# cc-ai/MUNIT

Measured on AMD Instinct MI355X. Metric: images/sec (gen_update+dis_update) @256x256 bs=8, higher is better.
Workload: dtype f32; 1 GPU; config_256.yaml AdaINGen_double+MsImageDis dis_update+gen_update, 256x256, per-GPU batch 8, fp32; global_batch=8, parallelism=dp1, gen_state=1

## Files before the change

munit_amd/csrc/conv_wgrad.hip:

```cpp
#include "common.h"
#include "wino.h"
#include <cstdlib>
#include <type_traits>

namespace {

struct WgradParams {
  const void* x;
  const void* dy;
  float* slab;
  float* bias_slab;
  int B, H, W, Cin, Hu, Wu, ups;
  int Ho, Wo, Cout;
  int KH, KW, stride, pad, reflect;
  int Ktot, M;
  int pix_per_split;
  long long dy_sb, dy_sh;
  int dy_sw;
  long long dy_off;
  int frame;
  unsigned x_bytes, dy_bytes;
  int ct;
  int x_bf16, dy_bf16;
};
// ... 868 lines not shown
  pl->bias_bytes = align_up((size_t)ns * Cout * sizeof(float), 256);
}

enum WgradForm {
  WG_REFUSED_BF16,
  WG_REFUSED_BF16_X,
  WG_BF16S_128,
  WG_BF16S_256,
  WG_REG_BF16,
  WG_REG_BF16_DY,
  WG_DMA,
  WG_CT1, WG_CT2,
  WG_FAST, WG_ALIGNED, WG_GENERIC
};
struct WgradChoice {
  WgradForm form;
  bool fast;
  long long x_bytes, dy_bytes;
};
WgradChoice wgrad_form(const WgradParams& p, const WgradPlan& pl, bool aligned) {
  WgradChoice c{};
  c.x_bytes = (long long)p.B * p.H * p.W * p.Cin * (p.x_bf16 ? 2 : 4);
  c.dy_bytes = (long long)p.B * p.dy_sb * (p.dy_bf16 ? 2 : 4);
  const bool any_bf16 = p.x_bf16 || p.dy_bf16;
  const bool fast_any = aligned && (p.Cout % 4 == 0) && c.x_bytes < (1ll << 31) && c.dy_bytes < (1ll << 31) &&
                        (long long)p.B * p.H * p.W < (1ll << 23) && (any_bf16 || !MUNIT_ENV_FLAG("MUNIT_DEBUG_NO_FAST_WGRAD"));
  const bool fast = c.fast = fast_any && !p.frame;
  if (any_bf16) {
    const bool dma_ok = p.x_bf16 && p.dy_bf16 && p.Cin % 128 == 0 && p.Cout % 8 == 0 && p.Ho + p.Wo <= DMA_MAX_HW;
    if (!fast && !(fast_any && dma_ok)) c.form = WG_REFUSED_BF16;
    else if (dma_ok && !MUNIT_ENV_FLAG("MUNIT_DEBUG_NO_WGRAD_DMA")) c.form = pl.bc == 256 ? WG_BF16S_256 : WG_BF16S_128;
    else if (p.x_bf16 && p.dy_bf16) c.form = WG_REG_BF16;
    else if (p.dy_bf16) c.form = WG_REG_BF16_DY;
    else c.form = WG_REFUSED_BF16_X;
  } else if (fast && p.ct == 0 && pl.bc == 128 && p.Cin % 128 == 0 && p.Ho + p.Wo <= DMA_MAX_HW &&
             !MUNIT_ENV_FLAG("MUNIT_DEBUG_NO_WGRAD_DMA")) {
    c.form = WG_DMA;
  } else if (fast && p.ct == 1) {
    c.form = WG_CT1;
  } else if (fast && p.ct == 2) {
    c.form = WG_CT2;
  } else {
    c.form = fast ? WG_FAST : aligned ? WG_ALIGNED : WG_GENERIC;
  }
  return c;
}

#define WGRAD_LAUNCH(...)                                                                                         \
  do {                                                                                                            \
    if (pl.bc == 64) hipLaunchKernelGGL((conv_wgrad_kernel<64, __VA_ARGS__>), grid, dim3(WTHR), 0, st, p);        \
    else hipLaunchKernelGGL((conv_wgrad_kernel<128, __VA_ARGS__>), grid, dim3(WTHR), 0, st, p);                   \
  } while (0)

int run_wgrad(WgradParams p, const WgradPlan& pl, bool aligned, float* dw, float* db, float beta, float beta_b,
              void* ws, hipStream_t st) {
  p.slab = reinterpret_cast<float*>(ws);
  p.bias_slab = db ? reinterpret_cast<float*>(reinterpret_cast<char*>(ws) + pl.slab_bytes) : nullptr;
  p.pix_per_split = pl.pix_per_split;
  dim3 grid((unsigned)pl.k_tiles, (unsigned)pl.c_tiles, (unsigned)pl.nsplit);
  const WgradChoice ch = wgrad_form(p, pl, aligned);
  p.x_bytes = ch.fast ? (unsigned)ch.x_bytes : 0u;
  p.dy_bytes = ch.fast ? (unsigned)ch.dy_bytes : 0u;
  switch (ch.form) {
    case WG_REFUSED_BF16:
      munit_set_error("conv2d_wgrad: bf16 tensors need Cin %% 4 == 0, Cout %% 4 == 0, tensors below 2 GiB and B*H*W < 2^23");
      return MUNIT_ERR_ARG;
    case WG_REFUSED_BF16_X:
      munit_set_error("conv2d_wgrad: bf16 x with fp32 dy exists for the 3-channel image head only");
      return MUNIT_ERR_ARG;
    case WG_BF16S_128:
    case WG_BF16S_256: {
      int pps = (cdiv(p.M, pl.nsplit) + BS_WP - 1) / BS_WP * BS_WP;
      p.pix_per_split = pps;
      const int ns = cdiv(p.M, pps);
      if (ch.form == WG_BF16S_256) {
        dim3 g2((unsigned)(p.Ktot / 256), (unsigned)(p.Cout / 256), (unsigned)ns);
        hipLaunchKernelGGL(conv_wgrad_bf16s_kernel<2>, g2, dim3(WTHR), 0, st, p);
      } else {
        dim3 g2((unsigned)cdiv(p.Ktot, 128), (unsigned)cdiv(p.Cout, 128), (unsigned)ns);
        hipLaunchKernelGGL(conv_wgrad_bf16s_kernel<1>, g2, dim3(WTHR), 0, st, p);
      }
      MUNIT_CHECK_LAUNCH("conv_wgrad_bf16s");
      const long long n = (long long)p.Cout * p.Ktot;
      const int blocks = (int)std::min<long long>((n + p.Cout + 255) / 256, 4096);
      hipLaunchKernelGGL(slab_reduce_kernel, dim3(blocks), dim3(256), 0, st, p.slab, dw, n, p.bias_slab, db, p.Cout,
                         ns, beta, beta_b);
      MUNIT_CHECK_LAUNCH("slab_reduce");
      return MUNIT_OK;
    }
    case WG_REG_BF16: WGRAD_LAUNCH(true, true, 1, true, true); break;
    case WG_REG_BF16_DY: WGRAD_LAUNCH(true, true, 0, false, true); break;
    case WG_DMA: hipLaunchKernelGGL((conv_wgrad_kernel<128, true, true, 3>), grid, dim3(WTHR), 0, st, p); break;
    case WG_CT1: WGRAD_LAUNCH(true, true, 1); break;
    case WG_CT2: WGRAD_LAUNCH(true, true, 2); break;
    case WG_FAST: WGRAD_LAUNCH(true, true); break;
    case WG_ALIGNED: WGRAD_LAUNCH(true, false); break;
    case WG_GENERIC: WGRAD_LAUNCH(false, false); break;
  }
  MUNIT_CHECK_LAUNCH("conv_wgrad");
  const long long n = (long long)p.Cout * p.Ktot;
  if (pl.nsplit >= 32 && n + p.Cout <= 64 * 2048) {
    hipLaunchKernelGGL(slab_reduce_wide_kernel, dim3(cdiv(n + p.Cout, 64)), dim3(1024), 0, st, p.slab, dw, n,
                       p.bias_slab, db, p.Cout, pl.nsplit, beta, beta_b);
    MUNIT_CHECK_LAUNCH("slab_reduce_wide");
    return MUNIT_OK;
  }
  const int blocks = (int)std::min<long long>((n + p.Cout + 255) / 256, 4096);
  hipLaunchKernelGGL(slab_reduce_kernel, dim3(blocks), dim3(256), 0, st, p.slab, dw, n, p.bias_slab, db, p.Cout,
                     pl.nsplit, beta, beta_b);
  MUNIT_CHECK_LAUNCH("slab_reduce");
  return MUNIT_OK;
}

bool cin3_padded_ok(const munit_conv_desc* d) {
  return d->Cin == 3 && d->Cout % 4 == 0 && d->upsample == 0 && !MUNIT_ENV_FLAG("MUNIT_DEBUG_NO_CIN3_PAD");
}

bool bf16s_big_tile(const munit_conv_desc* d, int Ho, int Wo) {
  if (MUNIT_ENV_FLAG("MUNIT_DEBUG_NO_WGRAD_BIG_TILE") || MUNIT_ENV_FLAG("MUNIT_DEBUG_NO_WGRAD_DMA")) return false;
  if (d->in_dtype != MUNIT_DTYPE_BF16 || d->out_dtype != MUNIT_DTYPE_BF16) return false;
  if (d->Cin % 256 != 0 || d->Cout % 256 != 0 || Ho + Wo > DMA_MAX_HW) return false;
  const long long tiles = (long long)(d->KH * d->KW * d->Cin / 256) * (d->Cout / 256);
  const long long M = (long long)d->B * Ho * Wo;
  return tiles <= 256 && M * tiles >= 256ll * 1024;
}

bool subpixel_wgrad_ok(const munit_conv_desc* d) {
  const bool f32 = d->in_dtype == MUNIT_DTYPE_F32 && d->out_dtype == MUNIT_DTYPE_F32;
  const bool b16 = d->in_dtype == MUNIT_DTYPE_BF16 && d->out_dtype == MUNIT_DTYPE_BF16 && d->Cin % 128 == 0 &&
                   d->Cout % 8 == 0 && 2 * (d->H + d->W) <= DMA_MAX_HW && !MUNIT_ENV_FLAG("MUNIT_DEBUG_NO_WGRAD_DMA");
  return (f32 || b16) && d->upsample == 1 && d->KH == 5 && d->KW == 5 && d->pad == 2 && d->stride == 1 &&
         d->pad_mode == MUNIT_PAD_REFLECT && d->Cin % 4 == 0 && d->H >= 3 && d->W >= 3 &&
         !MUNIT_ENV_FLAG("MUNIT_DEBUG_NO_SUBPIXEL");
}

struct SubpixelPlan {
  WgradPlan phase, frame;
  size_t dwc_bytes, slab_bytes;
  bool wino;
  int ring;
};
void plan_subpixel(const munit_conv_desc* d, SubpixelPlan* sp) {
  const bool aligned = d->Cin % 4 == 0;
  plan_launch(d->B * (d->H - 2) * (d->W - 2), 9 * d->Cin, d->Cout, aligned, &sp->phase);
  const int Ho = 2 * d->H, Wo = 2 * d->W;
  sp->wino = d->compute == MUNIT_COMPUTE_F32 && d->in_dtype == MUNIT_DTYPE_F32 && d->out_dtype == MUNIT_DTYPE_F32 && d->H >= 4 &&
             d->W >= 4 && munit_wino_wgrad_ok(d->B, d->H, d->W, d->Cin, d->Cout) &&
             (long long)d->B * 4 * d->H * d->W * d->Cout < (1ll << 29);
  sp->ring = sp->wino ? 1 : 2;
  plan_launch(d->B * (2 * sp->ring * Wo + 2 * sp->ring * (Ho - 2 * sp->ring)), 25 * d->Cin, d->Cout, aligned, &sp->frame);
  sp->dwc_bytes = align_up((size_t)4 * d->Cout * 9 * d->Cin * sizeof(float), 256);
  sp->slab_bytes = std::max(sp->phase.slab_bytes + sp->phase.bias_bytes, sp->frame.slab_bytes + sp->frame.bias_bytes);
  if (sp->wino)
    sp->slab_bytes = std::max(sp->slab_bytes, munit_wino_wgrad_workspace((long long)d->B * (d->H / 2) * (d->W / 2), d->Cin, d->Cout, 4));
}

bool wino_wgrad_layer(const munit_conv_desc* d) {
  return d->compute == MUNIT_COMPUTE_F32 && d->in_dtype == MUNIT_DTYPE_F32 && d->out_dtype == MUNIT_DTYPE_F32 && d->KH == 3 &&
         d->KW == 3 && d->stride == 1 && d->pad == 1 && d->upsample == 0 && munit_wino_wgrad_ok(d->B, d->H, d->W, d->Cin, d->Cout);
}
long long s2_tiles(const munit_conv_desc* d) { return (long long)d->B * cdiv(d->H / 2, 3) * cdiv(d->W / 2, 3); }
bool wino_s2_wgrad_layer(const munit_conv_desc* d) {
  return d->compute == MUNIT_COMPUTE_F32 && d->in_dtype == MUNIT_DTYPE_F32 && d->out_dtype == MUNIT_DTYPE_F32 && d->KH == 4 &&
         d->KW == 4 && d->stride == 2 && d->pad == 1 && d->upsample == 0 && d->H >= 4 && d->W >= 4 &&
         munit_wino_wgrad_ok(d->B, d->H, d->W, d->Cin, d->Cout) && !MUNIT_ENV_FLAG("MUNIT_DEBUG_NO_WINOGRAD_S2") &&
         s2_tiles(d) >= (getenv("MUNIT_WINO_S2_MIN_BLOCKS") ? 1 : 512);
}

enum WgradRoute { WGR_WINO_S2, WGR_WINO, WGR_SMALL, WGR_SUBPIXEL, WGR_CIN3, WGR_GENERIC };
struct WgradRoutePlan {
  int rc;
  WgradRoute route;
  int Ho, Wo;
  bool aligned;
  SubpixelPlan sp;
  WgradPlan gen;
  size_t x4_bytes, dw4_bytes;
  size_t ws_bytes;
};
WgradRoutePlan plan_wgrad(const munit_conv_desc* d) {
  WgradRoutePlan pl{};
  pl.rc = munit_conv2d_out_hw(d, &pl.Ho, &pl.Wo);
  if (pl.rc) return pl;
  pl.route = wino_s2_wgrad_layer(d) ? WGR_WINO_S2 : wino_wgrad_layer(d) ? WGR_WINO : munit_small_wgrad_ok(d) ? WGR_SMALL
             : subpixel_wgrad_ok(d) ? WGR_SUBPIXEL : cin3_padded_ok(d) ? WGR_CIN3 : WGR_GENERIC;
  pl.aligned = pl.route == WGR_CIN3 || d->Cin % 4 == 0;
  switch (pl.route) {
    case WGR_WINO_S2: pl.ws_bytes = munit_wino_wgrad_workspace(s2_tiles(d), d->Cin, d->Cout, 4); break;
    case WGR_WINO: pl.ws_bytes = munit_wino_wgrad_workspace((long long)d->B * (d->H / 2) * (d->W / 2), d->Cin, d->Cout, 1); break;
    case WGR_SMALL: pl.ws_bytes = munit_small_wgrad_workspace(d, pl.Ho); break;
    case WGR_SUBPIXEL:
      plan_subpixel(d, &pl.sp);
      pl.ws_bytes = pl.sp.dwc_bytes + pl.sp.slab_bytes;
      break;
    case WGR_CIN3:
      plan_launch(d->B * pl.Ho * pl.Wo, d->KH * d->KW * 4, d->Cout, true, &pl.gen);
      pl.x4_bytes = align_up((size_t)d->B * d->H * d->W * 4 * sizeof(float), 256);
      pl.dw4_bytes = align_up((size_t)d->Cout * d->KH * d->KW * 4 * sizeof(float), 256);
      pl.ws_bytes = pl.x4_bytes + pl.dw4_bytes + pl.gen.slab_bytes + pl.gen.bias_bytes;
      break;
    case WGR_GENERIC:
      plan_launch(d->B * pl.Ho * pl.Wo, d->KH * d->KW * d->Cin, d->Cout, pl.aligned, &pl.gen, bf16s_big_tile(d, pl.Ho, pl.Wo));
      pl.ws_bytes = pl.gen.slab_bytes + pl.gen.bias_bytes;
      break;
  }
  return pl;
}

WgradParams wgrad_params(const munit_conv_desc* d, int Ho, int Wo) {
  WgradParams p{};
  p.x_bf16 = d->in_dtype == MUNIT_DTYPE_BF16; p.dy_bf16 = d->out_dtype == MUNIT_DTYPE_BF16;
  p.B = d->B; p.H = d->H; p.W = d->W; p.Cin = d->Cin;
  p.ups = d->upsample; p.Hu = d->H << p.ups; p.Wu = d->W << p.ups;
  p.Ho = Ho; p.Wo = Wo; p.Cout = d->Cout;
  p.KH = d->KH; p.KW = d->KW; p.stride = d->stride; p.pad = d->pad;
  p.reflect = d->pad_mode == MUNIT_PAD_REFLECT;
  p.ct = d->compute;
  p.Ktot = d->KH * d->KW * d->Cin; p.M = d->B * Ho * Wo;
  p.dy_sw = d->Cout; p.dy_sh = (long long)Wo * d->Cout; p.dy_sb = (long long)Ho * Wo * d->Cout; p.dy_off = 0;
  return p;
}
WinoWgradParams wino_wgrad_params(const munit_conv_desc* d, int Ho, int Wo, WgradRoute route, const void* x, const void* dy) {
  WinoWgradParams q{};
  q.x = reinterpret_cast<const float*>(x); q.dy = reinterpret_cast<const float*>(dy);
  q.x_bytes = (unsigned)((size_t)d->B * d->H * d->W * d->Cin * 4); q.dy_bytes = (unsigned)((size_t)d->B * Ho * Wo * d->Cout * 4);
  q.dy_sw = d->Cout; q.dy_sh = (long long)Wo * d->Cout; q.dy_sb = (long long)Ho * Wo * d->Cout;
  q.B = d->B; q.H = d->H; q.W = d->W; q.Cin = d->Cin; q.Cout = d->Cout;
  q.reflect = d->pad_mode == MUNIT_PAD_REFLECT;
  q.th = d->H / 2; q.tw = d->W / 2; q.phases = 4;
  if (route == WGR_WINO_S2) {
    q.th = cdiv(Ho, 3); q.tw = cdiv(Wo, 3);
    q.s2 = 1; q.Ho = Ho; q.Wo = Wo;
  } else if (route == WGR_WINO) {
    q.xo = -1; q.phases = 1;
  } else {
    q.dy_sw *= 2; q.dy_sh *= 2; q.dy_prow = (long long)Wo * d->Cout; q.dy_pcol = d->Cout;
    q.reflect = 2; q.xo = -1; q.ring_mask = 1;
  }
  return q;
}
WgradParams subpixel_frame_params(const WgradParams& p, const munit_conv_desc* d, const SubpixelPlan& sp, int Ho, int Wo) {
  WgradParams f = p;
  f.frame = sp.ring;
  f.M = d->B * (2 * sp.ring * Wo + 2 * sp.ring * (Ho - 2 * sp.ring));
  return f;
}
WgradParams subpixel_phase_params(const WgradParams& p, const munit_conv_desc* d, int Wo, int ph) {
  const int a = ph >> 1, b = ph & 1;
  WgradParams q = p;
  q.ups = 0; q.Hu = d->H; q.Wu = d->W;
  q.Ho = d->H - 2; q.Wo = d->W - 2;
  q.KH = 3; q.KW = 3; q.pad = 0; q.reflect = 0;
  q.Ktot = 9 * d->Cin; q.M = d->B * q.Ho * q.Wo;
  q.dy_sw = 2 * d->Cout; q.dy_sh = (long long)2 * Wo * d->Cout;
  q.dy_off = ((long long)(2 + a) * Wo + 2 + b) * d->Cout;
  return q;
}
WgradParams cin3_params(const WgradParams& p, const munit_conv_desc* d) {
  WgradParams q = p;
  q.Cin = 4; q.Ktot = d->KH * d->KW * 4; q.x_bf16 = 0;
  q.ct = 0;
  return q;
}
const char* wgrad_refusal(WgradForm f) {
  if (f == WG_REFUSED_BF16) return "refused: bf16 tensors need Cin % 4 == 0, Cout % 4 == 0, tensors below 2 GiB and B*H*W < 2^23";
  if (f == WG_REFUSED_BF16_X) return "refused: bf16 x with fp32 dy exists for the 3-channel image head only";
  return nullptr;
}
}

extern "C" size_t munit_conv2d_wgrad_workspace_bytes(const munit_conv_desc* d) {
  const WgradRoutePlan pl = plan_wgrad(d);
  return pl.rc ? 0 : pl.ws_bytes;
}

extern "C" double munit_conv2d_executed_flops(const munit_conv_desc* d, int pass) {
  if (pass == MUNIT_PASS_FWD || pass == MUNIT_PASS_DGRAD) return munit_igemm_executed_flops(d, pass);
  if (pass != MUNIT_PASS_WGRAD) return 0.0;
  const WgradRoutePlan pl = plan_wgrad(d);
  if (pl.rc) return 0.0;
  const int Ho = pl.Ho, Wo = pl.Wo;
  const double cc = 2.0 * d->Cin * d->Cout;
  switch (pl.route) {
    case WGR_WINO: return cc * d->B * (d->H / 2) * (d->W / 2) * 16;
    case WGR_WINO_S2: return 4 * cc * (double)s2_tiles(d) * 16;
    case WGR_SUBPIXEL:
      if (pl.sp.wino) return cc * d->B * ((double)d->H * d->W * 4 * 4 + (2.0 * Wo + 2.0 * (Ho - 2)) * 25);
      return cc * d->B * ((double)(d->H - 2) * (d->W - 2) * 4 * 9 + (4.0 * Wo + 4.0 * (Ho - 4)) * 25);
    case WGR_CIN3: return 2.0 * 4 * d->Cout * d->B * Ho * Wo * d->KH * d->KW;
    default: return cc * d->B * Ho * Wo * d->KH * d->KW;
  }
}

extern "C" const char* munit_conv2d_kernel_name(const munit_conv_desc* d, int pass) {
  if (pass == MUNIT_PASS_FWD || pass == MUNIT_PASS_DGRAD) return munit_igemm_kernel_name(d, pass);
  if (pass != MUNIT_PASS_WGRAD) return "invalid";
  const WgradRoutePlan pl = plan_wgrad(d);
  if (pl.rc) return "invalid";
  const int Ho = pl.Ho, Wo = pl.Wo;
  const bool x_bf16 = d->in_dtype == MUNIT_DTYPE_BF16, dy_bf16 = d->out_dtype == MUNIT_DTYPE_BF16;
  const WgradParams p = wgrad_params(d, Ho, Wo);
  switch (pl.route) {
    case WGR_WINO_S2:
    case WGR_WINO: {
      const WinoWgradVariant v = munit_wino_wgrad_variant(wino_wgrad_params(d, Ho, Wo, pl.route, nullptr, nullptr));
      if (!v.s2) return v.fast ? "conv_wino_wgrad_kernel<false, true, false> + wino_wgrad_reduce_kernel"
                               : "conv_wino_wgrad_kernel<false, false, false> + wino_wgrad_reduce_kernel";
      return v.fast ? "conv_wino_wgrad_kernel<true, true, false> + wino_wgrad_reduce_kernel"
                    : v.ring ? "conv_wino_wgrad_kernel<true, false, true> + wino_wgrad_reduce_kernel"
                             : "conv_wino_wgrad_kernel<true, false, false> + wino_wgrad_reduce_kernel";
    }
    case WGR_SMALL:
      if (dy_bf16) return "refused: the 3-channel image head has an fp32 dy";
      if (!munit_small_wgrad_pk()) return x_bf16 ? "conv_lanes_wgrad_kernel<bf16_t>" : "conv_lanes_wgrad_kernel";
      return x_bf16 ? "conv_lanes_wgrad_pk_kernel<bf16_t>" : "conv_lanes_wgrad_pk_kernel";
    case WGR_SUBPIXEL: {
      if (pl.sp.wino) return "conv_wino_wgrad_kernel<false, ., true> x4 sub-pixel phases + frame + reduce";
      const WgradForm fr = wgrad_form(subpixel_frame_params(p, d, pl.sp, Ho, Wo), pl.sp.frame, pl.aligned).form;
      const WgradForm ph = wgrad_form(subpixel_phase_params(p, d, Wo, 0), pl.sp.phase, pl.aligned).form;
      if (wgrad_refusal(fr)) return wgrad_refusal(fr);
      if (wgrad_refusal(ph)) return wgrad_refusal(ph);
      if (ph == WG_BF16S_128 && fr == WG_BF16S_128) return "conv_wgrad_bf16s_kernel<1> x4 sub-pixel phases + frame";
      if (x_bf16 || dy_bf16) return "invalid";
      if (ph == WG_CT1) return "conv_wgrad_kernel<.., 1> x4 sub-pixel phases + fp32 frame";
      if (ph == WG_CT2) return "conv_wgrad_kernel<.., 2> x4 sub-pixel phases + fp32 frame";
      return "conv_wgrad_kernel x4 sub-pixel phases + frame";
    }
    case WGR_CIN3:
      if (x_bf16) return "refused: 3-channel inputs are fp32";
      break;
    case WGR_GENERIC: break;
  }
  const WgradForm f = wgrad_form(pl.route == WGR_CIN3 ? cin3_params(p, d) : p, pl.gen, pl.aligned).form;
  if (wgrad_refusal(f)) return wgrad_refusal(f);
  if (pl.route == WGR_CIN3) return f == WG_REG_BF16_DY ? "conv_wgrad_kernel<.., 0, false, true> (3 input channels padded to 4, bf16 dy)"
                                                       : "conv_wgrad_kernel (3 input channels padded to 4)";
  switch (f) {
    case WG_BF16S_128: return "conv_wgrad_bf16s_kernel<1> + slab_reduce_kernel";
    case WG_BF16S_256: return "conv_wgrad_bf16s_kernel<2> + slab_reduce_kernel";
    case WG_REG_BF16: return "conv_wgrad_kernel<.., 1, true, true> + slab_reduce_kernel";
    case WG_REG_BF16_DY: return "conv_wgrad_kernel<.., 0, false, true> + slab_reduce_kernel";
    case WG_CT1: return "conv_wgrad_kernel<.., 1> + slab_reduce_kernel";
// ... 72 lines not shown
```

munit_amd/csrc/conv_wino.hip:

```cpp
#include "wino.h"
#include <algorithm>
#include <type_traits>

namespace {

constexpr int WT = 64;
constexpr int WNB = 64;
constexpr int WK = 8;
constexpr int VBUF = 16 * WT * WK;
constexpr int UBUF = 16 * WNB * WK;
constexpr int MLD = 36;
constexpr int WINO_SMEM = 16 * WT * MLD;
static_assert(WINO_SMEM >= 2 * VBUF, "operand buffers must fit");

typedef float f32x2 __attribute__((ext_vector_type(2)));

#ifdef WINO_STAMP
__device__ long long g_wino_stamps[8 * 8 * 4];
#define WSTAMP(i) do { const long long t_ = __builtin_amdgcn_s_memtime(); st_acc[i] += t_ - st_last; st_last = t_; } while (0)
#else
#define WSTAMP(i) do { } while (0)
#endif

__device__ inline float wino_act(float v, int act, float slope) {
// ... 482 lines not shown
        } else {
          const int sw = (int)p.dy_sw * 4, sh = (int)p.dy_sh * 4;
          if constexpr (S2) {
            const int y0 = (int)(p.dy_off + b * p.dy_sb) * 4 + 3 * ty * sh + 3 * tx * sw;
#pragma unroll
            for (int i = 0; i < 3; ++i)
#pragma unroll
              for (int j = 0; j < 3; ++j) {
                const bool ok = FAST || (3 * ty + i < p.Ho && 3 * tx + j < p.Wo);
                g[i * 3 + j][e] = __builtin_bit_cast(float, __builtin_amdgcn_raw_buffer_load_b32(
                    yres, ok ? ylane : 0x80000000u, ok ? y0 + i * sh + j * sw : 0, 0));
              }
          } else {
            const int y0 = (int)(p.dy_off + (phase >> 1) * p.dy_prow + (phase & 1) * p.dy_pcol + b * p.dy_sb) * 4 + 2 * ty * sh + 2 * tx * sw;
            if constexpr (RING) {
              const bool r0 = !((phase >> 1) == 0 && ty == 0), r1 = !((phase >> 1) == 1 && ty == p.th - 1);
              const bool c0 = !((phase & 1) == 0 && tx == 0), c1 = !((phase & 1) == 1 && tx == p.tw - 1);
              g[0][e] = __builtin_bit_cast(float, __builtin_amdgcn_raw_buffer_load_b32(yres, r0 && c0 ? ylane : 0x80000000u, y0, 0));
              g[1][e] = __builtin_bit_cast(float, __builtin_amdgcn_raw_buffer_load_b32(yres, r0 && c1 ? ylane : 0x80000000u, y0 + sw, 0));
              g[2][e] = __builtin_bit_cast(float, __builtin_amdgcn_raw_buffer_load_b32(yres, r1 && c0 ? ylane : 0x80000000u, y0 + sh, 0));
              g[3][e] = __builtin_bit_cast(float, __builtin_amdgcn_raw_buffer_load_b32(yres, r1 && c1 ? ylane : 0x80000000u, y0 + sh + sw, 0));
            } else {
              g[0][e] = __builtin_bit_cast(float, __builtin_amdgcn_raw_buffer_load_b32(yres, ylane, y0, 0));
              g[1][e] = __builtin_bit_cast(float, __builtin_amdgcn_raw_buffer_load_b32(yres, ylane, y0 + sw, 0));
              g[2][e] = __builtin_bit_cast(float, __builtin_amdgcn_raw_buffer_load_b32(yres, ylane, y0 + sh, 0));
              g[3][e] = __builtin_bit_cast(float, __builtin_amdgcn_raw_buffer_load_b32(yres, ylane, y0 + sh + sw, 0));
            }
          }
        }
      } else {
#pragma unroll
        for (int q = 0; q < 16; ++q) d[q][e] = 0.f;
#pragma unroll
        for (int q = 0; q < NG; ++q) g[q][e] = 0.f;
      }
    }
    cur_t += 8; cur_tx += 8;
    while (cur_tx >= p.tw) { cur_tx -= p.tw; if (++cur_ty >= p.th) { cur_ty = 0; ++cur_b; } }
  };
  const int wpos = (pair * 64 + (lane ^ ((pair & 1) << 4))) * 2;
  auto transform_store = [&](int buf) {
    if (xside) {
      float* V = smem + (2 + buf) * WG_BUF + wpos;
      f32x2 u[16];
#pragma unroll
      for (int j = 0; j < 4; ++j) {
        u[0 + j] = d[0 + j] - d[8 + j];
        u[4 + j] = d[4 + j] + d[8 + j];
        u[8 + j] = d[8 + j] - d[4 + j];
        u[12 + j] = d[4 + j] - d[12 + j];
      }
#pragma unroll
      for (int i = 0; i < 4; ++i) {
        *reinterpret_cast<f32x2*>(V + (i * 4 + 0) * WG_PLANE) = u[i * 4 + 0] - u[i * 4 + 2];
        *reinterpret_cast<f32x2*>(V + (i * 4 + 1) * WG_PLANE) = u[i * 4 + 1] + u[i * 4 + 2];
        *reinterpret_cast<f32x2*>(V + (i * 4 + 2) * WG_PLANE) = u[i * 4 + 2] - u[i * 4 + 1];
        *reinterpret_cast<f32x2*>(V + (i * 4 + 3) * WG_PLANE) = u[i * 4 + 1] - u[i * 4 + 3];
      }
    } else {
      float* E = smem + buf * WG_BUF + wpos;
      if constexpr (S2) {
        if (want_db) {
          const f32x2 sum = ((g[0] + g[1]) + (g[2] + g[3])) + ((g[4] + g[5]) + (g[6] + g[7])) + g[8];
          dbs += sum[0];
          dbs += sum[1];
        }
        f32x2 r[4][3];
#pragma unroll
        for (int j = 0; j < 3; ++j) {
          r[0][j] = g[j];
          r[1][j] = (g[j] + g[6 + j]) + g[3 + j];
          r[2][j] = (g[j] + g[6 + j]) - g[3 + j];
          r[3][j] = -g[6 + j];
        }
#pragma unroll
        for (int i = 0; i < 4; ++i) {
          *reinterpret_cast<f32x2*>(E + (i * 4 + 0) * WG_PLANE) = r[i][0];
          *reinterpret_cast<f32x2*>(E + (i * 4 + 1) * WG_PLANE) = (r[i][0] + r[i][2]) + r[i][1];
          *reinterpret_cast<f32x2*>(E + (i * 4 + 2) * WG_PLANE) = (r[i][0] + r[i][2]) - r[i][1];
          *reinterpret_cast<f32x2*>(E + (i * 4 + 3) * WG_PLANE) = -r[i][2];
        }
      } else {
        if (want_db) {
          const f32x2 sum = (g[0] + g[1]) + (g[2] + g[3]);
          dbs += sum[0];
          dbs += sum[1];
        }
        const f32x2 r[4][2] = {{g[0], g[1]}, {g[0] + g[2], g[1] + g[3]}, {g[0] - g[2], g[1] - g[3]}, {-g[2], -g[3]}};
#pragma unroll
        for (int i = 0; i < 4; ++i) {
          *reinterpret_cast<f32x2*>(E + (i * 4 + 0) * WG_PLANE) = r[i][0];
          *reinterpret_cast<f32x2*>(E + (i * 4 + 1) * WG_PLANE) = r[i][0] + r[i][1];
          *reinterpret_cast<f32x2*>(E + (i * 4 + 2) * WG_PLANE) = r[i][0] - r[i][1];
          *reinterpret_cast<f32x2*>(E + (i * 4 + 3) * WG_PLANE) = -r[i][1];
        }
      }
    }
  };

  f32x4 acc[2][4][4];
#pragma unroll
  for (int fq = 0; fq < 2; ++fq)
#pragma unroll
    for (int mt = 0; mt < 4; ++mt)
#pragma unroll
      for (int nt = 0; nt < 4; ++nt) acc[fq][mt][nt] = f32x4{0.f, 0.f, 0.f, 0.f};
  int fpos[2][4];
#pragma unroll
  for (int fq = 0; fq < 2; ++fq)
#pragma unroll
    for (int mt = 0; mt < 4; ++mt) {
      fpos[fq][mt] = (wave * 2 + fq) * WG_PLANE + ((lane >> 4) * 64 + ((mt * 16 + (lane & 15)) ^ (((lane >> 4) & 1) << 4))) * 2;
      asm("" : "+v"(fpos[fq][mt]));
    }
  auto compute = [&](int buf, int fq) {
    const float* Ef = smem + buf * WG_BUF;
    const float* Vf = smem + (2 + buf) * WG_BUF;
    f32x2 a[4], bb[4];
#pragma unroll
    for (int nt = 0; nt < 4; ++nt) bb[nt] = *reinterpret_cast<const f32x2*>(Vf + fpos[fq][nt]);
#pragma unroll
    for (int mt = 0; mt < 4; ++mt) a[mt] = *reinterpret_cast<const f32x2*>(Ef + fpos[fq][mt]);
#pragma unroll
    for (int t = 0; t < 2; ++t)
#pragma unroll
      for (int mt = 0; mt < 4; ++mt)
#pragma unroll
        for (int nt = 0; nt < 4; ++nt)
          acc[fq][mt][nt] = __builtin_amdgcn_mfma_f32_16x16x4f32(a[mt][t], bb[nt][t], acc[fq][mt][nt], 0, 0, 0);
  };

  if (nc > 0) {
    load_raw(0);
    transform_store(0);
    if (nc > 1) load_raw(1);
  }
  __syncthreads();
  for (int c = 0; c < nc; ++c) {
    const int cur = c & 1;
    const bool more = c + 1 < nc;
    if (more && wave < 4) {
      transform_store(cur ^ 1);
      if (c + 2 < nc) load_raw(c + 2);
    }
    compute(cur, 0);
    compute(cur, 1);
    if (more && wave >= 4) {
      transform_store(cur ^ 1);
      if (c + 2 < nc) load_raw(c + 2);
    }
    __syncthreads();
  }

  float* const sl = p.slab + ((long long)phase * p.ksplit + split) * 16 * p.Cout * p.Cin;
#pragma unroll
  for (int fq = 0; fq < 2; ++fq)
#pragma unroll
    for (int mt = 0; mt < 4; ++mt)
#pragma unroll
      for (int nt = 0; nt < 4; ++nt)
#pragma unroll
        for (int r = 0; r < 4; ++r)
          sl[((long long)(wave * 2 + fq) * p.Cout + cob * 64 + mt * 16 + 4 * (lane >> 4) + r) * p.Cin + cib * 64 + nt * 16 + (lane & 15)] =
              acc[fq][mt][nt][r];
  if (want_db_blk) {
    smem[wave * 64 + lane] = dbs;
    __syncthreads();
    if (wave == 0) {
      float s = 0.f;
#pragma unroll
      for (int w = 0; w < 8; ++w) s += smem[w * 64 + lane];
      p.db_part[(phase * p.ksplit + split) * p.Cout + cob * 64 + lane] = s;
    }
  }
}

__global__ void wino_wgrad_reduce_kernel(const float* __restrict__ slab, const float* __restrict__ db_part, float* __restrict__ dw,
                                         long long dw_phase, float* __restrict__ db, int Cout, int Cin, int ksplit, float beta,
                                         float beta_b, int pair_blocks, int s2) {
  if ((int)blockIdx.x >= pair_blocks) {
    const int co = (blockIdx.x - pair_blocks) * blockDim.x + threadIdx.x;
    if (co < Cout && blockIdx.y == 0) {
      float s = 0.f;
      for (int k = 0; k < ksplit * (s2 ? 1 : (int)gridDim.y); ++k) s += db_part[k * Cout + co];
      db[co] = beta_b == 0.f ? s : beta_b * db[co] + s;
    }
    return;
  }
  slab += (long long)blockIdx.y * ksplit * 16 * Cout * Cin;
  dw += blockIdx.y * dw_phase;
  const long long idx = (long long)blockIdx.x * blockDim.x + threadIdx.x;
  if (idx >= (long long)Cout * Cin) return;
  const int ci = (int)(idx % Cin), co = (int)(idx / Cin);
  const long long plane = (long long)Cout * Cin;
  float S[16];
#pragma unroll
  for (int f = 0; f < 16; ++f) S[f] = 0.f;
  for (int k = 0; k < ksplit; ++k) {
    const float* sp = slab + (long long)k * 16 * plane + idx;
#pragma unroll
    for (int f = 0; f < 16; ++f) S[f] += sp[f * plane];
  }
  if (s2) {
    const int r = blockIdx.y >> 1, sf = blockIdx.y & 1;
    float t[2][4];
#pragma unroll
    for (int j = 0; j < 4; ++j) {
      t[0][j] = S[j] + 0.5f * (S[4 + j] + S[8 + j]);
      t[1][j] = 0.5f * (S[4 + j] - S[8 + j]) + S[12 + j];
    }
#pragma unroll
    for (int a = 0; a < 2; ++a) {
      const float v[2] = {t[a][0] + 0.5f * (t[a][1] + t[a][2]), 0.5f * (t[a][1] - t[a][2]) + t[a][3]};
#pragma unroll
      for (int b = 0; b < 2; ++b) {
        float* o = dw - blockIdx.y * dw_phase + (((long long)co * 4 + 2 * a + r) * 4 + 2 * b + sf) * Cin + ci;
        *o = beta == 0.f ? v[b] : beta * *o + v[b];
      }
    }
    return;
  }
  float t[3][4];
#pragma unroll
  for (int j = 0; j < 4; ++j) {
    const float h = 0.5f * (S[4 + j] + S[8 + j]), m = 0.5f * (S[4 + j] - S[8 + j]);
    t[0][j] = S[j] + h;
    t[1][j] = m;
    t[2][j] = h + S[12 + j];
  }
#pragma unroll
  for (int r = 0; r < 3; ++r) {
    const float h = 0.5f * (t[r][1] + t[r][2]), m = 0.5f * (t[r][1] - t[r][2]);
    const float v[3] = {t[r][0] + h, m, h + t[r][3]};
#pragma unroll
    for (int s = 0; s < 3; ++s) {
      float* o = dw + (((long long)co * 3 + r) * 3 + s) * Cin + ci;
      *o = beta == 0.f ? v[s] : beta * *o + v[s];
    }
  }
}

}

#ifdef WINO_STAMP
extern "C" int munit_debug_wino_stamps(long long* host_out) {
  return hipMemcpyFromSymbol(host_out, HIP_SYMBOL(g_wino_stamps), sizeof(long long) * 8 * 8 * 4) == hipSuccess ? 0 : -1;
}
#endif

bool munit_wino_wgrad_ok(int B, int H, int W, int Cin, int Cout) {
  if (MUNIT_ENV_FLAG("MUNIT_DEBUG_NO_WINOGRAD") || MUNIT_ENV_FLAG("MUNIT_DEBUG_NO_WINOGRAD_WGRAD")) return false;
  return Cin % 64 == 0 && Cout % 64 == 0 && H % 2 == 0 && W % 2 == 0 && H >= 2 && W >= 2 &&
         (long long)B * H * W * std::max(Cin, Cout) < (1ll << 29);
}

int munit_wino_wgrad_splits(long long tiles, int Cin, int Cout, int phases) {
  const int chunks = cdiv(tiles, 8);
  const int pairs = (Cin / 64) * (Cout / 64) * std::max(1, phases);
  int ksplit = std::max(1, std::min(chunks, cdiv(256, pairs)));
  const int cps = cdiv(chunks, ksplit);
  return cdiv(chunks, cps);
}

size_t munit_wino_wgrad_workspace(long long tiles, int Cin, int Cout, int phases) {
  const size_t k = (size_t)munit_wino_wgrad_splits(tiles, Cin, Cout, phases) * std::max(1, phases);
  return align_up(k * 16 * Cin * Cout * sizeof(float), 256) + align_up(k * Cout * sizeof(float), 256);
}

WinoWgradVariant munit_wino_wgrad_variant(const WinoWgradParams& p) {
  const bool whole = (p.B * p.th * p.tw) % 8 == 0 && !MUNIT_ENV_FLAG("MUNIT_DEBUG_NO_WINO_WGRAD_FAST");
  if (p.s2) {
    const bool fast = whole && p.reflect && p.H % 6 == 0 && p.W % 6 == 0 && p.Ho % 3 == 0 && p.Wo % 3 == 0;
    return {true, fast, !fast && whole && p.reflect == 1 && p.H >= 2 && p.W >= 2};
  }
  const bool fast = whole && (p.xo == -1 ? (p.reflect && p.H >= 2 && p.W >= 2 && 2 * p.th <= p.H && 2 * p.tw <= p.W)
                                         : (p.xo >= 0 && 2 * (p.th - 1) + p.xo + 3 < p.H && 2 * (p.tw - 1) + p.xo + 3 < p.W));
  return {false, fast, p.ring_mask != 0};
}

int munit_wino_wgrad_launch(WinoWgradParams p, float* dw, long long dw_phase, float* db, float beta, float beta_b, void* ws,
                            hipStream_t st) {
  p.phases = std::max(1, p.phases);
  p.tiles = p.B * p.th * p.tw;
  p.ksplit = munit_wino_wgrad_splits(p.tiles, p.Cin, p.Cout, p.phases);
  p.cps = cdiv(cdiv(p.tiles, 8), p.ksplit);
  p.CB = p.Cin / 64; p.NB = p.Cout / 64;
  p.slab = reinterpret_cast<float*>(ws);
  float* db_part = reinterpret_cast<float*>(reinterpret_cast<char*>(ws) +
                                            align_up((size_t)p.ksplit * p.phases * 16 * p.Cin * p.Cout * sizeof(float), 256));
  p.db_part = db != nullptr ? db_part : nullptr;
  const dim3 grid((unsigned)(p.CB * p.NB * p.ksplit), (unsigned)p.phases);
  const WinoWgradVariant v = munit_wino_wgrad_variant(p);
  if (v.s2) {
    if (v.fast) hipLaunchKernelGGL((conv_wino_wgrad_kernel<true, true>), grid, dim3(512), 0, st, p);
    else if (v.ring) hipLaunchKernelGGL((conv_wino_wgrad_kernel<true, false, true>), grid, dim3(512), 0, st, p);
    else hipLaunchKernelGGL((conv_wino_wgrad_kernel<true, false>), grid, dim3(512), 0, st, p);
  } else if (v.ring) {
    MUNIT_CHECK_ARG(p.reflect == 2 && p.xo == -1 && p.phases == 4, "conv_wino_wgrad: ring_mask goes with the replicated edge and 4 phases");
    if (v.fast) hipLaunchKernelGGL((conv_wino_wgrad_kernel<false, true, true>), grid, dim3(512), 0, st, p);
    else hipLaunchKernelGGL((conv_wino_wgrad_kernel<false, false, true>), grid, dim3(512), 0, st, p);
  } else {
    MUNIT_CHECK_ARG(p.reflect != 2, "conv_wino_wgrad: the replicated edge goes with ring_mask");
    if (v.fast) hipLaunchKernelGGL((conv_wino_wgrad_kernel<false, true>), grid, dim3(512), 0, st, p);
    else hipLaunchKernelGGL((conv_wino_wgrad_kernel<false, false>), grid, dim3(512), 0, st, p);
  }
  MUNIT_CHECK_LAUNCH("conv_wino_wgrad");
  const int pair_blocks = cdiv((long long)p.Cout * p.Cin, 256);
  const int bias_blocks = db != nullptr ? cdiv(p.Cout, 256) : 0;
  hipLaunchKernelGGL(wino_wgrad_reduce_kernel, dim3((unsigned)(pair_blocks + bias_blocks), (unsigned)p.phases), dim3(256), 0, st, p.slab,
                     db_part, dw, dw_phase, db, p.Cout, p.Cin, p.ksplit, beta, beta_b, pair_blocks, p.s2);
  MUNIT_CHECK_LAUNCH("wino_wgrad_reduce");
  return MUNIT_OK;
}

bool munit_wino_ok(int B, int H, int W, int K, int N) {
  if (MUNIT_ENV_FLAG("MUNIT_DEBUG_NO_WINOGRAD")) return false;
  return K % 8 == 0 && N % 64 == 0 && H % 2 == 0 && W % 2 == 0 && H >= 2 && W >= 2 &&
         (long long)B * H * W * K < (1ll << 29) && (long long)B * H * W * N < (1ll << 40);
}

int munit_wino_launch(const WinoParams& p, hipStream_t st) {
  const bool lin = p.s2 == 1 || p.s2 == 2;
  const long long blocks = lin ? (long long)cdiv((long long)p.B * p.th * p.tw, 64) * p.NB : (long long)p.B * p.bth * p.btw * p.NB;
  MUNIT_CHECK_ARG(blocks > 0 && blocks < (1ll << 31), "conv_wino: bad grid");
  const dim3 grid((unsigned)blocks, (unsigned)std::max(1, p.phases));
  if (p.s2 == 1) {
    if (p.mode == 0) hipLaunchKernelGGL((conv_wino_kernel<0, 1>), grid, dim3(512), 0, st, p);
    else hipLaunchKernelGGL((conv_wino_kernel<1, 1>), grid, dim3(512), 0, st, p);
    MUNIT_CHECK_LAUNCH("conv_wino_s2");
    return MUNIT_OK;
  }
  if (p.s2 == 3) {
    hipLaunchKernelGGL((conv_wino_kernel<1, 3>), grid, dim3(512), 0, st, p);
    MUNIT_CHECK_LAUNCH("conv_wino_up_dgrad");
    return MUNIT_OK;
  }
  if (p.s2 == 2) {
    if (p.mode == 0) hipLaunchKernelGGL((conv_wino_kernel<0, 2>), grid, dim3(512), 0, st, p);
    else hipLaunchKernelGGL((conv_wino_kernel<1, 2>), grid, dim3(512), 0, st, p);
    MUNIT_CHECK_LAUNCH("conv_wino_s2_dgrad");
    return MUNIT_OK;
  }
  if (p.mode == 0) hipLaunchKernelGGL(conv_wino_kernel<0>, grid, dim3(512), 0, st, p);
  else if (p.mode == 1) hipLaunchKernelGGL(conv_wino_kernel<1>, grid, dim3(512), 0, st, p);
  else hipLaunchKernelGGL(conv_wino_kernel<2>, grid, dim3(512), 0, st, p);
  MUNIT_CHECK_LAUNCH("conv_wino");
  return MUNIT_OK;
}
```

munit_amd/csrc/wino.h:

```cpp
#pragma once
#include "common.h"

__host__ __device__ inline long long wino_image_elems(int K, int N) { return 16ll * K * N; }

__device__ inline float wino_u_of_g(const float (&g)[3][3], int f) {
  const int fi = f >> 2, fj = f & 3;
  float t[3];
#pragma unroll
  for (int s = 0; s < 3; ++s) {
    const float a = g[0][s], b = g[1][s], cc = g[2][s];
    t[s] = fi == 0 ? a : fi == 1 ? 0.5f * ((a + cc) + b) : fi == 2 ? 0.5f * ((a + cc) - b) : cc;
  }
  return fj == 0 ? t[0] : fj == 1 ? 0.5f * ((t[0] + t[2]) + t[1]) : fj == 2 ? 0.5f * ((t[0] + t[2]) - t[1]) : t[2];
}

__device__ inline void wino_item_index(long long j, int N, int& k, int& no) {
  const int NB = N >> 6;
  const int w = (int)(j & 511);
  const int e = w & 1, ntl = (w >> 1) & 1, l = (w >> 2) & 63, h = w >> 8;
  const long long rest = j >> 9;
  const int nb = (int)(rest % NB), c = (int)(rest / NB);
  k = c * 8 + 2 * (l >> 4) + e;
  no = nb * 64 + (2 * h + ntl) * 16 + (l & 15);
}
// ... 10 lines not shown
#pragma unroll
  for (int r = 0; r < 3; ++r)
#pragma unroll
    for (int s = 0; s < 3; ++s)
      g[r][s] = dgrad ? w[(((long long)k * 3 + (2 - r)) * 3 + (2 - s)) * Cin + no] : w[(((long long)no * 3 + r) * 3 + s) * Cin + k];
  wino_store_item(img, j, g);
}

__device__ inline void wino_s2_weight_item(const float* __restrict__ w, float* __restrict__ img, int Cout, int Cin, long long j) {
  int k, no;
  wino_item_index(j, Cout, k, no);
  const int phase = k / Cin, ci = k - phase * Cin, r = phase >> 1, sft = phase & 1;
  float g[2][2];
#pragma unroll
  for (int a = 0; a < 2; ++a)
#pragma unroll
    for (int b = 0; b < 2; ++b) g[a][b] = w[(((long long)no * 4 + 2 * a + r) * 4 + 2 * b + sft) * Cin + ci];
  float t[4][2];
#pragma unroll
  for (int b = 0; b < 2; ++b) {
    t[0][b] = g[0][b];
    t[1][b] = 0.5f * (g[0][b] + g[1][b]);
    t[2][b] = 0.5f * (g[0][b] - g[1][b]);
    t[3][b] = g[1][b];
  }
  float* o = img + (j >> 9) * (16 * 512) + (j & 511);
#pragma unroll
  for (int fi = 0; fi < 4; ++fi) {
    o[(fi * 4 + 0) * 512] = t[fi][0];
    o[(fi * 4 + 1) * 512] = 0.5f * (t[fi][0] + t[fi][1]);
    o[(fi * 4 + 2) * 512] = 0.5f * (t[fi][0] - t[fi][1]);
    o[(fi * 4 + 3) * 512] = t[fi][1];
  }
}

__device__ inline void wino_s2_dgrad_weight_item(const float* __restrict__ w, float* __restrict__ img, int Cout, int Cin, long long j) {
  const long long per = (long long)Cin * Cout;
  const int phase = (int)(j / per), ph = phase >> 1, pw = phase & 1;
  const long long jj = j - phase * per;
  int k, no;
  wino_item_index(jj, Cin, k, no);
  float g[2][2];
#pragma unroll
  for (int a = 0; a < 2; ++a)
#pragma unroll
    for (int b = 0; b < 2; ++b) g[a][b] = w[(((long long)k * 4 + 2 * (1 - a) + ph) * 4 + 2 * (1 - b) + pw) * Cin + no];
  float t[4][2];
#pragma unroll
  for (int b = 0; b < 2; ++b) {
    t[0][b] = g[0][b];
    t[1][b] = 0.5f * (g[0][b] + g[1][b]);
    t[2][b] = 0.5f * (g[0][b] - g[1][b]);
    t[3][b] = g[1][b];
  }
  float* o = img + phase * wino_image_elems(Cout, Cin) + (jj >> 9) * (16 * 512) + (jj & 511);
#pragma unroll
  for (int fi = 0; fi < 4; ++fi) {
    o[(fi * 4 + 0) * 512] = t[fi][0];
    o[(fi * 4 + 1) * 512] = 0.5f * (t[fi][0] + t[fi][1]);
    o[(fi * 4 + 2) * 512] = 0.5f * (t[fi][0] - t[fi][1]);
    o[(fi * 4 + 3) * 512] = t[fi][1];
  }
}

__device__ inline void wino_subpixel_dgrad_weight_item(const float* __restrict__ w, float* __restrict__ img, int Cout, int Cin, long long j) {
  int k, no;
  wino_item_index(j, Cin, k, no);
  const int ph = k / Cout, co = k - ph * Cout, a = ph >> 1, b = ph & 1;
  float g[3][3];
#pragma unroll
  for (int r = 0; r < 3; ++r)
#pragma unroll
    for (int sft = 0; sft < 3; ++sft) {
      const int dh = 2 - r, dw = 2 - sft;
      const int h0 = a == 0 ? (dh == 0 ? 0 : dh == 1 ? 2 : 4) : (dh == 0 ? 0 : dh == 1 ? 1 : 3);
      const int hn = a == 0 ? (dh == 2 ? 1 : 2) : (dh == 0 ? 1 : 2);
      const int w0 = b == 0 ? (dw == 0 ? 0 : dw == 1 ? 2 : 4) : (dw == 0 ? 0 : dw == 1 ? 1 : 3);
      const int wn = b == 0 ? (dw == 2 ? 1 : 2) : (dw == 0 ? 1 : 2);
      float sum = 0.f;
      for (int kh = h0; kh < h0 + hn; ++kh)
        for (int kw = w0; kw < w0 + wn; ++kw) sum += w[(((long long)co * 5 + kh) * 5 + kw) * Cin + no];
      g[r][sft] = sum;
    }
  wino_store_item(img, j, g);
}

__device__ inline void wino_subpixel_weight_item(const float* __restrict__ w, float* __restrict__ img, int Cout, int Cin, long long j) {
  const long long per = (long long)Cin * Cout;
  const int ph = (int)(j / per), a = ph >> 1, b = ph & 1;
  int k, no;
  wino_item_index(j - ph * per, Cout, k, no);
  float g[3][3];
#pragma unroll
  for (int dh = 0; dh < 3; ++dh)
#pragma unroll
    for (int dw = 0; dw < 3; ++dw) {
      const int h0 = a == 0 ? (dh == 0 ? 0 : dh == 1 ? 2 : 4) : (dh == 0 ? 0 : dh == 1 ? 1 : 3);
      const int hn = a == 0 ? (dh == 2 ? 1 : 2) : (dh == 0 ? 1 : 2);
      const int w0 = b == 0 ? (dw == 0 ? 0 : dw == 1 ? 2 : 4) : (dw == 0 ? 0 : dw == 1 ? 1 : 3);
      const int wn = b == 0 ? (dw == 2 ? 1 : 2) : (dw == 0 ? 1 : 2);
      float s = 0.f;
      for (int kh = h0; kh < h0 + hn; ++kh)
        for (int kw = w0; kw < w0 + wn; ++kw) s += w[(((long long)no * 5 + kh) * 5 + kw) * Cin + k];
      g[dh][dw] = s;
    }
  wino_store_item(img + ph * wino_image_elems(Cin, Cout), j - ph * per, g);
}

struct WinoParams {
  const float* x;
  const float* u;
  const float* bias;
  const float* add;
  float* y;
  long long y_sb, y_sh, y_sw;
  long long u_phase, y_prow, y_pcol;
  int phases;
  unsigned x_bytes;
  int B, H, W, K, N;
  int xc, cpp;
  int s2, Ho, Wo;
  int mode;
  int edge;
  int th, tw;
  int bth, btw;
  int NB;
  int act;
  float slope;
};

bool munit_wino_ok(int B, int H, int W, int K, int N);
int munit_wino_launch(const WinoParams& p, hipStream_t st);

struct WinoWgradParams {
  const float* x;
  const float* dy;
  float* slab;
  float* db_part;
  unsigned x_bytes, dy_bytes;
  long long dy_sb, dy_sh, dy_sw, dy_off;
  long long dy_prow, dy_pcol;
  int B, H, W, Cin, Cout;
  int reflect;
  int ring_mask;
  int xo;
  int th, tw, tiles;
  int cps;
  int CB, NB, ksplit;
  int phases;
  int s2, Ho, Wo;
};
bool munit_wino_wgrad_ok(int B, int H, int W, int Cin, int Cout);
int munit_wino_wgrad_splits(long long tiles, int Cin, int Cout, int phases);
size_t munit_wino_wgrad_workspace(long long tiles, int Cin, int Cout, int phases);
struct WinoWgradVariant { bool s2, fast, ring; };
WinoWgradVariant munit_wino_wgrad_variant(const WinoWgradParams& p);
int munit_wino_wgrad_launch(WinoWgradParams p, float* dw, long long dw_phase, float* db, float beta, float beta_b, void* ws,
                            hipStream_t st);
```

Measured before the change: 79.10 images/s.

## Apply Winograd output transform in wgrad kernel epilogue before split reduction

Each Winograd wgrad block now stages its accumulators through shared memory and applies the inverse output transform itself. It writes 9 (or 4 for stride-2) spatial taps per split instead of 16 Winograd-domain planes. The reduce kernel then only sums the splits with vectorized float4 loads and writes dw directly. This shrinks slab traffic and workspace and simplifies the reduction. The cost is extra shared-memory staging and two more barriers in the main kernel's epilogue.

```diff
diff --git a/munit_amd/csrc/conv_wgrad.hip b/munit_amd/csrc/conv_wgrad.hip
--- a/munit_amd/csrc/conv_wgrad.hip
+++ b/munit_amd/csrc/conv_wgrad.hip
@@ -1044,7 +1044,7 @@
   sp->dwc_bytes = align_up((size_t)4 * d->Cout * 9 * d->Cin * sizeof(float), 256);
   sp->slab_bytes = std::max(sp->phase.slab_bytes + sp->phase.bias_bytes, sp->frame.slab_bytes + sp->frame.bias_bytes);
   if (sp->wino)
-    sp->slab_bytes = std::max(sp->slab_bytes, munit_wino_wgrad_workspace((long long)d->B * (d->H / 2) * (d->W / 2), d->Cin, d->Cout, 4));
+    sp->slab_bytes = std::max(sp->slab_bytes, munit_wino_wgrad_workspace((long long)d->B * (d->H / 2) * (d->W / 2), d->Cin, d->Cout, 4, false));
 }
 
 bool wino_wgrad_layer(const munit_conv_desc* d) {
@@ -1078,8 +1078,8 @@
              : subpixel_wgrad_ok(d) ? WGR_SUBPIXEL : cin3_padded_ok(d) ? WGR_CIN3 : WGR_GENERIC;
   pl.aligned = pl.route == WGR_CIN3 || d->Cin % 4 == 0;
   switch (pl.route) {
-    case WGR_WINO_S2: pl.ws_bytes = munit_wino_wgrad_workspace(s2_tiles(d), d->Cin, d->Cout, 4); break;
-    case WGR_WINO: pl.ws_bytes = munit_wino_wgrad_workspace((long long)d->B * (d->H / 2) * (d->W / 2), d->Cin, d->Cout, 1); break;
+    case WGR_WINO_S2: pl.ws_bytes = munit_wino_wgrad_workspace(s2_tiles(d), d->Cin, d->Cout, 4, true); break;
+    case WGR_WINO: pl.ws_bytes = munit_wino_wgrad_workspace((long long)d->B * (d->H / 2) * (d->W / 2), d->Cin, d->Cout, 1, false); break;
     case WGR_SMALL: pl.ws_bytes = munit_small_wgrad_workspace(d, pl.Ho); break;
     case WGR_SUBPIXEL:
       plan_subpixel(d, &pl.sp);
diff --git a/munit_amd/csrc/conv_wino.hip b/munit_amd/csrc/conv_wino.hip
--- a/munit_amd/csrc/conv_wino.hip
+++ b/munit_amd/csrc/conv_wino.hip
@@ -658,18 +658,60 @@
     __syncthreads();
   }
 
-  float* const sl = p.slab + ((long long)phase * p.ksplit + split) * 16 * p.Cout * p.Cin;
-#pragma unroll
-  for (int fq = 0; fq < 2; ++fq)
-#pragma unroll
-    for (int mt = 0; mt < 4; ++mt)
-#pragma unroll
-      for (int nt = 0; nt < 4; ++nt)
-#pragma unroll
-        for (int r = 0; r < 4; ++r)
-          sl[((long long)(wave * 2 + fq) * p.Cout + cob * 64 + mt * 16 + 4 * (lane >> 4) + r) * p.Cin + cib * 64 + nt * 16 + (lane & 15)] =
-              acc[fq][mt][nt][r];
+  constexpr int TAPS = S2 ? 4 : 9;
+  float* const sl = p.slab + ((long long)phase * p.ksplit + split) * TAPS * p.Cout * p.Cin;
+  const int rco = tid >> 4, rc4 = tid & 15;
+  const float* const rp = smem + rco * 64 + ((4 * rc4) ^ (((rco >> 2) & 3) << 4));
+#pragma unroll
+  for (int h = 0; h < 2; ++h) {
+    if (h) __syncthreads();
+#pragma unroll
+    for (int fq = 0; fq < 2; ++fq)
+#pragma unroll
+      for (int m = 0; m < 2; ++m)
+#pragma unroll
+        for (int nt = 0; nt < 4; ++nt)
+#pragma unroll
+          for (int r = 0; r < 4; ++r)
+            smem[((wave * 2 + fq) * 32 + m * 16 + 4 * (lane >> 4) + r) * 64 + ((nt ^ (lane >> 4)) * 16 + (lane & 15))] =
+                acc[fq][2 * h + m][nt][r];
+    __syncthreads();
+    f32x4 S[16];
+#pragma unroll
+    for (int f = 0; f < 16; ++f) S[f] = *reinterpret_cast<const f32x4*>(rp + f * (32 * 64));
+    float* const o = sl + (long long)(cob * 64 + h * 32 + rco) * TAPS * p.Cin + cib * 64 + 4 * rc4;
+    if constexpr (S2) {
+      f32x4 t[2][4];
+#pragma unroll
+      for (int j = 0; j < 4; ++j) {
+        t[0][j] = S[j] + 0.5f * (S[4 + j] + S[8 + j]);
+        t[1][j] = 0.5f * (S[4 + j] - S[8 + j]) + S[12 + j];
+      }
+#pragma unroll
+      for (int a = 0; a < 2; ++a) {
+        *reinterpret_cast<f32x4*>(o + (2 * a + 0) * p.Cin) = t[a][0] + 0.5f * (t[a][1] + t[a][2]);
+        *reinterpret_cast<f32x4*>(o + (2 * a + 1) * p.Cin) = 0.5f * (t[a][1] - t[a][2]) + t[a][3];
+      }
+    } else {
+      f32x4 t[3][4];
+#pragma unroll
+      for (int j = 0; j < 4; ++j) {
+        const f32x4 hs = 0.5f * (S[4 + j] + S[8 + j]), ms = 0.5f * (S[4 + j] - S[8 + j]);
+        t[0][j] = S[j] + hs;
+        t[1][j] = ms;
+        t[2][j] = hs + S[12 + j];
+      }
+#pragma unroll
+      for (int r = 0; r < 3; ++r) {
+        const f32x4 hs = 0.5f * (t[r][1] + t[r][2]), ms = 0.5f * (t[r][1] - t[r][2]);
+        *reinterpret_cast<f32x4*>(o + (3 * r + 0) * p.Cin) = t[r][0] + hs;
+        *reinterpret_cast<f32x4*>(o + (3 * r + 1) * p.Cin) = ms;
+        *reinterpret_cast<f32x4*>(o + (3 * r + 2) * p.Cin) = hs + t[r][3];
+      }
+    }
+  }
   if (want_db_blk) {
+    __syncthreads();
     smem[wave * 64 + lane] = dbs;
     __syncthreads();
     if (wave == 0) {
@@ -693,56 +735,28 @@
     }
     return;
   }
-  slab += (long long)blockIdx.y * ksplit * 16 * Cout * Cin;
-  dw += blockIdx.y * dw_phase;
+  const int c4n = Cin >> 2;
+  const long long n4 = (long long)Cout * (s2 ? 4 : 9) * c4n;
   const long long idx = (long long)blockIdx.x * blockDim.x + threadIdx.x;
-  if (idx >= (long long)Cout * Cin) return;
-  const int ci = (int)(idx % Cin), co = (int)(idx / Cin);
-  const long long plane = (long long)Cout * Cin;
-  float S[16];
-#pragma unroll
-  for (int f = 0; f < 16; ++f) S[f] = 0.f;
-  for (int k = 0; k < ksplit; ++k) {
-    const float* sp = slab + (long long)k * 16 * plane + idx;
-#pragma unroll
-    for (int f = 0; f < 16; ++f) S[f] += sp[f * plane];
-  }
+  if (idx >= n4) return;
+  const f32x4* sp = reinterpret_cast<const f32x4*>(slab) + (long long)blockIdx.y * ksplit * n4 + idx;
+  f32x4 v = sp[0];
+#pragma unroll 4
+  for (int k = 1; k < ksplit; ++k) v += sp[k * n4];
+  float* o;
   if (s2) {
+    const int ci4 = (int)(idx % c4n), ct = (int)(idx / c4n), co = ct >> 2, a = (ct >> 1) & 1, b = ct & 1;
     const int r = blockIdx.y >> 1, sf = blockIdx.y & 1;
-    float t[2][4];
-#pragma unroll
-    for (int j = 0; j < 4; ++j) {
-      t[0][j] = S[j] + 0.5f * (S[4 + j] + S[8 + j]);
-      t[1][j] = 0.5f * (S[4 + j] - S[8 + j]) + S[12 + j];
-    }
-#pragma unroll
-    for (int a = 0; a < 2; ++a) {
-      const float v[2] = {t[a][0] + 0.5f * (t[a][1] + t[a][2]), 0.5f * (t[a][1] - t[a][2]) + t[a][3]};
-#pragma unroll
-      for (int b = 0; b < 2; ++b) {
-        float* o = dw - blockIdx.y * dw_phase + (((long long)co * 4 + 2 * a + r) * 4 + 2 * b + sf) * Cin + ci;
-        *o = beta == 0.f ? v[b] : beta * *o + v[b];
-      }
-    }
-    return;
-  }
-  float t[3][4];
-#pragma unroll
-  for (int j = 0; j < 4; ++j) {
-    const float h = 0.5f * (S[4 + j] + S[8 + j]), m = 0.5f * (S[4 + j] - S[8 + j]);
-    t[0][j] = S[j] + h;
-    t[1][j] = m;
-    t[2][j] = h + S[12 + j];
-  }
-#pragma unroll
-  for (int r = 0; r < 3; ++r) {
-    const float h = 0.5f * (t[r][1] + t[r][2]), m = 0.5f * (t[r][1] - t[r][2]);
-    const float v[3] = {t[r][0] + h, m, h + t[r][3]};
-#pragma unroll
-    for (int s = 0; s < 3; ++s) {
-      float* o = dw + (((long long)co * 3 + r) * 3 + s) * Cin + ci;
-      *o = beta == 0.f ? v[s] : beta * *o + v[s];
-    }
+    o = dw + (((long long)co * 4 + 2 * a + r) * 4 + 2 * b + sf) * Cin + 4 * ci4;
+  } else {
+    o = dw + blockIdx.y * dw_phase + idx * 4;
+  }
+  if ((reinterpret_cast<uintptr_t>(o) & 15) == 0) {
+    f32x4* o4 = reinterpret_cast<f32x4*>(o);
+    *o4 = beta == 0.f ? v : beta * *o4 + v;
+  } else {
+#pragma unroll
+    for (int e = 0; e < 4; ++e) o[e] = beta == 0.f ? v[e] : beta * o[e] + v[e];
   }
 }
 
@@ -768,9 +782,14 @@
   return cdiv(chunks, cps);
 }
 
-size_t munit_wino_wgrad_workspace(long long tiles, int Cin, int Cout, int phases) {
-  const size_t k = (size_t)munit_wino_wgrad_splits(tiles, Cin, Cout, phases) * std::max(1, phases);
-  return align_up(k * 16 * Cin * Cout * sizeof(float), 256) + align_up(k * Cout * sizeof(float), 256);
+static size_t wino_wgrad_slab_bytes(int ksplit, int phases, int Cin, int Cout, bool s2) {
+  return align_up((size_t)ksplit * std::max(1, phases) * (s2 ? 4 : 9) * Cin * Cout * sizeof(float), 256);
+}
+
+size_t munit_wino_wgrad_workspace(long long tiles, int Cin, int Cout, int phases, bool s2) {
+  const int ksplit = munit_wino_wgrad_splits(tiles, Cin, Cout, phases);
+  return wino_wgrad_slab_bytes(ksplit, phases, Cin, Cout, s2) +
+         align_up((size_t)ksplit * std::max(1, phases) * Cout * sizeof(float), 256);
 }
 
 WinoWgradVariant munit_wino_wgrad_variant(const WinoWgradParams& p) {
@@ -793,7 +812,7 @@
   p.CB = p.Cin / 64; p.NB = p.Cout / 64;
   p.slab = reinterpret_cast<float*>(ws);
   float* db_part = reinterpret_cast<float*>(reinterpret_cast<char*>(ws) +
-                                            align_up((size_t)p.ksplit * p.phases * 16 * p.Cin * p.Cout * sizeof(float), 256));
+                                            wino_wgrad_slab_bytes(p.ksplit, p.phases, p.Cin, p.Cout, p.s2 != 0));
   p.db_part = db != nullptr ? db_part : nullptr;
   const dim3 grid((unsigned)(p.CB * p.NB * p.ksplit), (unsigned)p.phases);
   const WinoWgradVariant v = munit_wino_wgrad_variant(p);
@@ -811,7 +830,7 @@
     else hipLaunchKernelGGL((conv_wino_wgrad_kernel<false, false>), grid, dim3(512), 0, st, p);
   }
   MUNIT_CHECK_LAUNCH("conv_wino_wgrad");
-  const int pair_blocks = cdiv((long long)p.Cout * p.Cin, 256);
+  const int pair_blocks = cdiv((long long)p.Cout * (p.s2 ? 4 : 9) * (p.Cin / 4), 256);
   const int bias_blocks = db != nullptr ? cdiv(p.Cout, 256) : 0;
   hipLaunchKernelGGL(wino_wgrad_reduce_kernel, dim3((unsigned)(pair_blocks + bias_blocks), (unsigned)p.phases), dim3(256), 0, st, p.slab,
                      db_part, dw, dw_phase, db, p.Cout, p.Cin, p.ksplit, beta, beta_b, pair_blocks, p.s2);
diff --git a/munit_amd/csrc/wino.h b/munit_amd/csrc/wino.h
--- a/munit_amd/csrc/wino.h
+++ b/munit_amd/csrc/wino.h
@@ -186,7 +186,7 @@
 };
 bool munit_wino_wgrad_ok(int B, int H, int W, int Cin, int Cout);
 int munit_wino_wgrad_splits(long long tiles, int Cin, int Cout, int phases);
-size_t munit_wino_wgrad_workspace(long long tiles, int Cin, int Cout, int phases);
+size_t munit_wino_wgrad_workspace(long long tiles, int Cin, int Cout, int phases, bool s2);
 struct WinoWgradVariant { bool s2, fast, ring; };
 WinoWgradVariant munit_wino_wgrad_variant(const WinoWgradParams& p);
 int munit_wino_wgrad_launch(WinoWgradParams p, float* dw, long long dw_phase, float* db, float beta, float beta_b, void* ws,
```

New measurement: 79.51 images/s (median of 6 runs). No clear change (+0.5%).
